# ingonyama-zk/blaze

Measured on AMD Instinct MI355X. Metric: BLS12-381 MSM/s at 2^26, higher is better.
Workload: dtype u32 registers holding 28-bit limbs (381-bit Fq, Montgomery)

## Files before the change

blaze_amd/_lib.py:

```python
from __future__ import annotations

import ctypes as C
import os

_HERE = os.path.dirname(os.path.abspath(__file__))
LIB_PATH = os.environ.get("BLAZE_HIP_LIB") or os.path.join(_HERE, "lib", "libblaze_hip.so")


class DriverClientError(Exception):

    VARIANTS = {
        1: "WriteError",
        2: "ReadError",
        3: "HBICAPNotReady",
        4: "InvalidPrimitiveParam",
        5: "CsvError",
        6: "LoadFailed",
        7: "FileError",
        8: "Unknown",
    }

    def __init__(self, code: int, message: str):
        self.code = code
        self.variant = self.VARIANTS.get(code, "Unknown")
# ... 131 lines not shown
    "blz_poseidon_raw_results": (C.c_int, [C.c_void_p, C.c_uint32, _u8p, C.c_size_t]),
    "blz_poseidon_result": (C.c_int, [C.c_void_p, C.c_uint32, _u8p, C.c_size_t, C.POINTER(C.c_uint32)]),
    "blz_poseidon_tree_device": (C.c_int, [C.c_void_p, C.c_void_p, C.c_size_t]),
    "blz_poseidon_counters": (C.c_int, [C.c_void_p, C.POINTER(C.c_uint32)]),
    "blz_poseidon_info": (C.c_int, [C.c_void_p, C.POINTER(C.c_uint64)]),
    "blz_poseidon_set_round_plan": (C.c_int, [C.c_void_p, C.c_int]),
    "blz_poseidon_prepare_round_plan": (C.c_int, [C.c_void_p, C.POINTER(C.c_uint32)]),
    "blz_poseidon_last_kernel_ms": (C.c_int, [C.c_void_p, C.POINTER(C.c_float)]),
    "blz_poseidon_stream": (C.c_int, [C.c_void_p, C.POINTER(C.c_void_p), C.POINTER(C.c_int)]),
    "blz_poseidon_reset": (C.c_int, [C.c_void_p]),
    "blz_device_malloc": (C.c_int, [C.c_int, C.c_size_t, C.POINTER(C.c_void_p)]),
    "blz_device_free": (C.c_int, [C.c_int, C.c_void_p]),
    "blz_host_malloc": (C.c_int, [C.c_int, C.c_size_t, C.POINTER(C.c_void_p)]),
    "blz_host_free": (C.c_int, [C.c_void_p]),
    "blz_memcpy_h2d": (C.c_int, [C.c_int, C.c_void_p, _u8p, C.c_size_t]),
    "blz_memcpy_d2h": (C.c_int, [C.c_int, _u8p, C.c_void_p, C.c_size_t]),
}
EXPORTED_SYMBOLS = tuple(_SIGS)
_AUX_SIGS = {
    "blz_synth_scalars": (C.c_int, [C.c_int, C.c_int, C.c_void_p, C.c_uint64, C.c_uint64]),
    "blz_synth_scalars_at": (C.c_int, [C.c_int, C.c_int, C.c_void_p, C.c_uint64, C.c_uint64, C.c_uint64]),
    "blz_synth_points": (C.c_int, [C.c_int, C.c_int, C.c_void_p, C.c_uint64, C.c_int, C.c_uint64]),
    "blz_synth_field_elements": (C.c_int, [C.c_int, C.c_void_p, C.c_uint64, C.c_uint64]),
    "blz_calib_mad_rate": (C.c_int, [C.c_int, C.c_uint32, C.POINTER(C.c_double)]),
    "blz_test_msm_stall": (C.c_int, [C.c_void_p, C.c_uint32, C.POINTER(C.c_void_p)]),
    "blz_test_ntt_stall": (C.c_int, [C.c_void_p, C.c_uint32, C.POINTER(C.c_void_p)]),
    "blz_test_stall_release": (C.c_int, [C.c_void_p]),
    "blz_test_field_op": (C.c_int, [C.c_int, C.c_int, C.c_int, C.c_int, _u8p, _u8p, _u8p, C.c_size_t]),
    "blz_test_ec_op": (C.c_int, [C.c_int, C.c_int, C.c_int, _u8p, _u8p, _u8p, _u8p, _u8p, C.c_size_t]),
    "blz_test_msm_tail_plan": (C.c_int, [C.c_int, C.c_int, C.c_uint32, C.c_int, C.c_int, C.c_int, C.c_int, C.c_int, C.POINTER(C.c_uint32), C.POINTER(C.c_uint8),
                                         C.c_char_p, C.c_size_t]),
    "blz_test_msm_sort_plan": (C.c_int, [C.c_int, C.c_int, C.c_uint32, C.c_int, C.c_int, C.c_int, C.c_int, C.c_int, C.c_int, C.c_int, C.c_int, C.c_int,
                                         C.c_char_p, C.c_size_t]),
    "blz_test_law_layout": (C.c_int, [C.c_int, C.c_int, C.c_int, C.POINTER(C.c_uint32)]),
    "blz_test_law_op": (C.c_int, [C.c_int, C.c_int, C.c_int, C.c_int, C.c_int, C.c_int, C.c_uint32, C.c_uint32, _u8p, _u8p, C.c_size_t]),
    "blz_test_rr_layout": (C.c_int, [C.c_int, C.c_int, C.POINTER(C.c_uint32)]),
    "blz_test_rr_op": (C.c_int, [C.c_int, C.c_int, C.c_int, C.c_int, C.c_int, _u8p, _u8p, C.c_size_t]),
    "blz_test_sort_fits_beside": (C.c_int, [C.c_int, C.c_int, C.c_int, C.c_int]),
    "blz_test_poseidon_permute": (C.c_int, [C.c_int, C.c_int, _u8p, C.c_size_t, C.c_int, _u8p, _u8p, C.c_size_t]),
    "blz_test_poseidon_hash": (C.c_int, [C.c_int, C.c_int, _u8p, C.c_size_t, C.c_int, _u8p, _u8p, C.c_size_t]),
    "blz_test_poseidon_hash_plan": (C.c_int, [C.c_int, C.c_int, _u8p, C.c_size_t, C.c_int, _u8p, _u8p, C.c_size_t, C.POINTER(C.c_uint32)]),
    "blz_test_poseidon_tree_check": (C.c_int, [C.c_int, C.c_int, _u8p, C.c_size_t, C.c_int, C.c_uint32, C.c_void_p, C.c_void_p, C.POINTER(C.c_uint64)]),
}
AUX_EXPORTED_SYMBOLS = tuple(_AUX_SIGS)


def lib():
    global _lib
    if _lib is None:
        if not os.path.exists(LIB_PATH):
            raise RuntimeError(
                f"{LIB_PATH} is missing: build it with `make -C blaze_amd/csrc` "
                "(or __graft_entry__.build()); blaze_amd has no CPU fallback"
            )
        L = C.CDLL(LIB_PATH, mode=C.RTLD_GLOBAL)
        for name, (res, args) in _SIGS.items():
            fn = getattr(L, name)
            fn.restype = res
            fn.argtypes = args
        _lib = L
    return _lib


def aux():
    global _aux
    if _aux is None:
# ... 98 lines not shown
```

blaze_amd/csrc/msm_digits.hip.hpp:

```cpp
#pragma once
#include <hip/hip_runtime.h>
#include <cstdint>

namespace blz {

template <int SW>
struct ScalarWords {
    uint32_t s[SW];
    __device__ __forceinline__ void load(const uint32_t* scalars, uint32_t p) {
        if constexpr (SW == 8) {
            const uint4* q = reinterpret_cast<const uint4*>(scalars) + 2 * (size_t)p;
            uint4 a = q[0], b = q[1];
            s[0] = a.x; s[1] = a.y; s[2] = a.z; s[3] = a.w; s[4] = b.x; s[5] = b.y; s[6] = b.z; s[7] = b.w;
        } else if constexpr (SW == 2) {
            const uint2 a = reinterpret_cast<const uint2*>(scalars)[p];
            s[0] = a.x; s[1] = a.y;
        } else {
            s[0] = scalars[p];
        }
    }
    __device__ __forceinline__ int next(int c, uint32_t mask, uint32_t half, uint32_t& carry) {
        uint32_t v = (s[0] & mask) + carry;
#pragma unroll
        for (int i = 0; i + 1 < SW; ++i) s[i] = __builtin_amdgcn_alignbit(s[i + 1], s[i], c);
        s[SW - 1] >>= c;
        if (v > half) { carry = 1; return (int)v - (int)(half << 1); }
        carry = 0;
        return (int)v;
    }
};


#define BLZ_SW_DISPATCH(sbits, ...)                                   \
    do {                                                              \
        if ((sbits) == 256) { constexpr int SW = 8; __VA_ARGS__; }    \
        else if ((sbits) == 64) { constexpr int SW = 2; __VA_ARGS__; } \
        else { constexpr int SW = 1; __VA_ARGS__; }                   \
    } while (0)

}
```

blaze_amd/csrc/msm_engine.hpp:

```cpp
#pragma once
#include "common.hpp"
#include <optional>

namespace blz {

constexpr int MSM_MAX_W = 96;
constexpr uint64_t MSM_MAX_ENTRIES = (1ull << 32) - (1ull << 26);
struct MsmPlan {
    uint32_t npts = 0;
    int sbits = 256;
    int c = 0;
    int W = 0;
    uint8_t width[MSM_MAX_W] = {};
    uint32_t boff[MSM_MAX_W + 1] = {};
    uint32_t Bw = 0;
    int Wv = 0;
    uint64_t G = 0;
    uint32_t L = 0;
    bool table = false;
    int ebits = 0;
    int base_bit = 0;
    double cost = 0;
};
MsmPlan make_plan(uint32_t npts, int sbits, int ebits, int force_c);
// ... 125 lines not shown
    bool can_accept() const;
    MsmPlan plan_for(uint32_t npts, int sbits) const;
    int points_to_mont(const void* d_raw, void* d_mont, uint32_t npts);
    int points_to_mont_even(const void* d_raw, void* d_mont, uint32_t nq);
    int check_precompute(const void* d_raw, uint64_t nelem, uint32_t* flag, hipStream_t st);
    int build_table(const void* d_raw, void* d_table, uint32_t npts, int c, int W, int base_shift, void* scratch, uint32_t* flag,
                    hipStream_t st);
    size_t table_scratch_bytes(int W) const;
    int run(const void* d_points_mont, const void* d_scalars, uint32_t npts, int sbits, int* slot, int table_c = 0, int bit_lo = 0,
            int bit_hi = 0);
    MsmPlan plan_for_range(uint32_t npts, int bit_lo, int bit_hi) const;
    int finish(int slot, uint8_t* out);
    int combine_partials(const uint8_t* partials, size_t count, uint8_t* out, bool on_device);
    int sync_all();
};

struct MsmStep {
    int slot;
    MsmSlot& S;
    int piece;
    const MsmPlan& P;
    MsmEngine::SortBufs& B;
    hipStream_t stream, sort_stream;
};

int msm_points_from_mont(int format_id, const void* d_mont, void* d_raw, uint64_t npts, hipStream_t st);
int msm_points_all_canonical(int format_id, const void* d_raw, uint64_t npts, uint32_t* flag, hipStream_t st);
int copy_words_to_pinned(void* host_pinned, const void* d_src, uint32_t dwords, hipStream_t st);
size_t fq_bytes(int curve);
size_t mont_point_bytes(int curve);
int msm_sort_stage(MsmEngine& E, const MsmStep& C, const void* d_scalars, uint32_t np);
void launch_zero(void* p, size_t n16, hipStream_t st);
bool msm_sort3_ok(const MsmPlan& P, int sbits);
int msm_sort3_max_vgprs(bool table);
int msm_sort3_max_lds(bool table);
bool msm_sort_fits_beside(int av, int sv, int al, int sl);
bool msm_sort_tiny_ok(const MsmPlan& P, uint32_t npts, int sbits);

struct MsmCurveOps {
    int (*points_to_mont)(MsmEngine&, const void* d_raw, void* d_mont, uint32_t npts);
    int (*emit_infinity)(MsmEngine&, int slot);
    int (*run_accumulate)(MsmEngine&, const MsmStep& C, const void* d_pts, uint32_t max_units);
    int (*merge_buckets)(MsmEngine&, const MsmStep& C);
    int (*run_reduce)(MsmEngine&, const MsmStep& C, const void* sums, const void* unit_off);
    TailTraits tail;
    int (*accumulate_vgprs)();
    int (*accumulate_lds)();
    int (*build_table)(MsmEngine&, const void* d_raw, void* d_table, uint32_t npts, int c, int W, int base_shift, void* scratch,
                       uint32_t* flag, hipStream_t st);
    size_t (*table_scratch_bytes)(int W);
    int (*combine)(MsmEngine&, const uint8_t* partials, size_t count, uint8_t* out, bool on_device);
    int (*points_to_mont_even)(MsmEngine&, const void* d_raw, void* d_mont, uint32_t nq);
    int (*check_precompute)(MsmEngine&, const void* d_raw, uint64_t nelem, uint32_t* flag, hipStream_t st);
    int (*points_from_mont)(const void* d_mont, void* d_raw, uint64_t npts, hipStream_t st);
    int (*points_all_canonical)(const void* d_raw, uint64_t npts, uint32_t* flag, hipStream_t st);
};
const MsmCurveOps& msm_ops_bls377();
const MsmCurveOps& msm_ops_bls381();
const MsmCurveOps& msm_ops_bn254();
const MsmCurveOps& msm_ops_bn254_w32();
const MsmCurveOps* msm_ops_for(int curve, int repr = 0);

}
```

blaze_amd/csrc/msm_sort3.hip:

```cpp
#include "msm_sort.hpp"
#include "msm_digits.hip.hpp"

namespace blz {

constexpr int S3_THREADS = 256;
constexpr int S3_SH1 = 14;
constexpr int S3_SH2 = 7;
#ifndef BLZ_S3_T
#define BLZ_S3_T 8
#endif
constexpr int S3_T = BLZ_S3_T;
constexpr int S3_PB = S3_THREADS * S3_T;
constexpr uint32_t S3_SLICE2 = 4096;
constexpr int S3_T2 = S3_SLICE2 / S3_THREADS;
constexpr int S3_T3 = 28;
constexpr uint32_t S3_R3 = S3_THREADS * S3_T3;
constexpr uint32_t S3_MAXNB1 = 2048;
constexpr uint32_t S3_CNT_PTS = 16384;
constexpr uint32_t S3T_IMG = 12288;

struct S3Geom {
    int W, prio;
    uint32_t NB1;
    uint8_t width[MSM_MAX_W];
    uint16_t bitoff[MSM_MAX_W];
    uint16_t binoff1[MSM_MAX_W + 1];
    static constexpr bool TABLE = false;
    static constexpr uint32_t HIST1 = S3_MAXNB1;
    using Win = int;
    __device__ int cw(int w) const { return width[w]; }
    __device__ uint32_t first_bin(int w) const { return binoff1[w]; }
    __device__ static constexpr uint32_t shift1() { return S3_SH1; }
    static constexpr uint32_t bits3() { return S3_SH2; }
    __device__ static uint32_t index1(uint32_t p, uint32_t, uint32_t) { return p; }
    __device__ static uint32_t rem1(uint32_t rem) { return rem; }
    struct L2 {
        int prio;
        using Lo = uint8_t;
        static constexpr uint32_t TAB2 = 128;
        static constexpr uint32_t KY_D = 8, KY_R = 16;
        static constexpr uint32_t LO_MASK = 127u;
        __device__ static constexpr uint32_t shift2() { return S3_SH2; }
        __device__ static constexpr uint32_t bits2() { return S3_SH1 - S3_SH2; }
        __device__ static uint32_t low2(uint32_t r, uint32_t) { return r & 127u; }
        __device__ static uint32_t index2(uint32_t iw) { return iw; }
    };
    L2 l2() const { return L2{prio}; }
};

struct S3TGeom {
    int W, prio, c;
    uint32_t sh1, b2, b3, xs, NB1;
    static constexpr bool TABLE = true;
    static constexpr uint32_t HIST1 = 256;
    using Win = uint32_t;
    __device__ int cw(int) const { return c; }
    __device__ static constexpr uint32_t first_bin(int) { return 0; }
    __device__ uint32_t shift1() const { return sh1; }
    uint32_t bits3() const { return b3; }
    __device__ uint32_t index1(uint32_t p, uint32_t w, uint32_t rem) const { return (p * (uint32_t)W + w) | (xs ? (rem & 1u) << 30 : 0u); }
    __device__ uint32_t rem1(uint32_t rem) const { return rem >> xs; }
    using L2 = S3TGeom;
    using Lo = uint16_t;
    static constexpr uint32_t TAB2 = 256;
    static constexpr uint32_t KY_D = 10, KY_R = 18;
    static constexpr uint32_t LO_MASK = 0x3ffu;
    __device__ uint32_t shift2() const { return b3 - xs; }
    __device__ uint32_t bits2() const { return b2; }
    __device__ uint32_t low2(uint32_t r, uint32_t iw) const {
        const uint32_t lomask = (1u << shift2()) - 1u;
        return xs ? ((r & lomask) << 1) | ((iw >> 30) & 1u) : (r & lomask);
    }
    __device__ static uint32_t index2(uint32_t iw) { return iw & 0xbfffffffu; }
    const L2& l2() const { return *this; }
};

__device__ __forceinline__ void s3_setprio(int p) {
    if (p >= 3) __builtin_amdgcn_s_setprio(3);
    else if (p == 2) __builtin_amdgcn_s_setprio(2);
    else if (p == 1) __builtin_amdgcn_s_setprio(1);
}

__device__ __forceinline__ uint32_t s3_wave_incl_scan(uint32_t v) {
    for (int o = 1; o < 64; o <<= 1) {
        uint32_t t = __shfl_up(v, o, 64);
        if ((threadIdx.x & 63u) >= (uint32_t)o) v += t;
    }
    return v;
}
__device__ __forceinline__ uint32_t s3_block_excl_scan(uint32_t v, uint32_t* wave_tot, uint32_t* total) {
    const uint32_t incl = s3_wave_incl_scan(v);
    if ((threadIdx.x & 63u) == 63u) wave_tot[threadIdx.x >> 6] = incl;
    __syncthreads();
    uint32_t wbase = 0;
    for (uint32_t q = 0; q < (threadIdx.x >> 6); ++q) wbase += wave_tot[q];
    *total = wave_tot[0] + wave_tot[1] + wave_tot[2] + wave_tot[3];
    return wbase + incl - v;
}

template <class Geom, int NW>
__global__ __launch_bounds__(S3_THREADS, 4) void k3_l1_count(const uint32_t* __restrict__ scalars, uint32_t npts, Geom g,
                                                            uint32_t* __restrict__ cnt1) {
    s3_setprio(g.prio);
    __shared__ uint32_t hist[Geom::HIST1];
    if constexpr (Geom::HIST1 == S3_THREADS) hist[threadIdx.x] = 0;
    else for (uint32_t i = threadIdx.x; i < g.NB1; i += S3_THREADS) hist[i] = 0;
    __syncthreads();
    const uint32_t base = blockIdx.x * S3_CNT_PTS;
    uint32_t end = base + S3_CNT_PTS;
    if (end > npts) end = npts;
    for (uint32_t p0 = base + threadIdx.x; p0 < end; p0 += 4 * S3_THREADS) {
        ScalarWords<NW> sw[4];
#pragma unroll
        for (int u = 0; u < 4; ++u) {
            const uint32_t p = p0 + u * S3_THREADS;
            sw[u].load(scalars, p < end ? p : p0);
        }
#pragma unroll
        for (int u = 0; u < 4; ++u) {
            if (p0 + u * S3_THREADS >= end) break;
            uint32_t carry = 0;
            for (int w = 0; w < g.W; ++w) {
                const int cw = g.cw(w);
                const int d = sw[u].next(cw, (1u << cw) - 1u, 1u << (cw - 1), carry);
                if (d != 0) {
                    const uint32_t b = (uint32_t)(d < 0 ? -d : d) - 1u;
                    atomicAdd(&hist[g.first_bin(w) + (b >> g.shift1())], 1u);
                }
            }
        }
    }
    __syncthreads();
    auto flush = [&](uint32_t i) {
        const uint32_t v = hist[i];
        if (v) atomicAdd(&cnt1[i], v);
    };
    if constexpr (Geom::HIST1 == S3_THREADS) { if (threadIdx.x < g.NB1) flush(threadIdx.x); }
    else for (uint32_t i = threadIdx.x; i < g.NB1; i += S3_THREADS) flush(i);
}

__global__ __launch_bounds__(S3_THREADS) void k3_scan_small(const uint32_t* __restrict__ cnt, uint32_t n, uint32_t* __restrict__ off,
                                                           uint32_t* __restrict__ cur, int prio) {
    s3_setprio(prio);
    __shared__ uint32_t wave_tot[4];
    uint32_t v[8], sum = 0;
    const uint32_t b0 = threadIdx.x * 8u;
#pragma unroll
    for (int k = 0; k < 8; ++k) {
        v[k] = b0 + k < n ? cnt[b0 + k] : 0u;
        sum += v[k];
    }
    uint32_t total;
    uint32_t run = s3_block_excl_scan(sum, wave_tot, &total);
#pragma unroll
    for (int k = 0; k < 8; ++k) {
        if (b0 + k < n) {
            off[b0 + k] = run;
            cur[b0 + k] = run;
        }
        run += v[k];
    }
    if (threadIdx.x == 0) off[n] = total;
}

template <class Geom, int NW>
__global__ __launch_bounds__(S3_THREADS, 4) void k3_l1_scatter(const uint32_t* __restrict__ scalars, uint32_t npts, Geom g,
                                                              uint32_t* __restrict__ cur1, uint32_t* __restrict__ o_idx,
                                                              uint16_t* __restrict__ o_rem) {
    s3_setprio(g.prio);
    extern __shared__ __attribute__((aligned(16))) uint32_t sh[];
    uint32_t* sc = sh;
    uint2* stage = reinterpret_cast<uint2*>(sh + NW * S3_PB);
    uint32_t* hist = sh + (NW + 2) * S3_PB;
    uint32_t* lstart = hist + 256;
    uint32_t* gbase = lstart + 256;
    __shared__ uint32_t wave_tot[4];
    const uint32_t tid = threadIdx.x;
    const uint32_t base = blockIdx.x * (uint32_t)S3_PB;
#pragma unroll
    for (int u = 0; u < S3_T; ++u) {
        const uint32_t p = base + u * S3_THREADS + tid;
        const uint32_t i = u * S3_THREADS + tid;
        if constexpr (NW == 8) {
            uint4 a = make_uint4(0, 0, 0, 0), b = make_uint4(0, 0, 0, 0);
            if (p < npts) {
                const uint4* q = reinterpret_cast<const uint4*>(scalars) + 2 * (size_t)p;
                a = q[0];
                b = q[1];
            }
            sc[0 * S3_PB + i] = a.x; sc[1 * S3_PB + i] = a.y; sc[2 * S3_PB + i] = a.z; sc[3 * S3_PB + i] = a.w;
            sc[4 * S3_PB + i] = b.x; sc[5 * S3_PB + i] = b.y; sc[6 * S3_PB + i] = b.z; sc[7 * S3_PB + i] = b.w;
        } else if constexpr (NW == 2) {
            uint2 a = make_uint2(0, 0);
            if (p < npts) a = reinterpret_cast<const uint2*>(scalars)[p];
            sc[0 * S3_PB + i] = a.x; sc[1 * S3_PB + i] = a.y;
        } else {
            sc[i] = p < npts ? scalars[p] : 0u;
        }
    }
    uint32_t carry = 0;
    using Win = typename Geom::Win;
    for (Win w = 0; w < (Win)g.W; ++w) {
        uint32_t cw, off, nb;
        if constexpr (Geom::TABLE) { cw = (uint32_t)g.c; off = w * cw; nb = g.NB1; }
        else { cw = g.width[w]; off = g.bitoff[w]; nb = (uint32_t)g.binoff1[w + 1] - (uint32_t)g.binoff1[w]; }
        const uint32_t sh1 = g.shift1(), lowmask = (1u << sh1) - 1u;
        const uint32_t j = off >> 5, shb = off & 31u, mask = (1u << cw) - 1u, half = 1u << (cw - 1);
        if (Geom::TABLE || tid < nb) hist[tid] = 0;
        __syncthreads();
        uint32_t key[S3_T], rk[S3_T];
#pragma unroll
        for (int u = 0; u < S3_T; ++u) {
            const uint32_t i = u * S3_THREADS + tid;
            const uint32_t lo = j < (uint32_t)NW ? sc[j * S3_PB + i] : 0u;
            const uint32_t hi = j + 1 < (uint32_t)NW ? sc[(j + 1) * S3_PB + i] : 0u;
            const uint32_t raw = (shb ? __builtin_amdgcn_alignbit(hi, lo, shb) : lo) & mask;
            const uint32_t v = raw + ((carry >> u) & 1u);
            int d;
            if (v > half) { d = (int)v - (int)(half << 1); carry |= 1u << u; }
            else { d = (int)v; carry &= ~(1u << u); }
            rk[u] = ~0u;
            key[u] = 0;
            if (d != 0 && base + i < npts) {
                const uint32_t b = (uint32_t)(d < 0 ? -d : d) - 1u;
                const uint32_t bin = b >> sh1;
                key[u] = (b & lowmask) | (bin << sh1) | (d < 0 ? 0x80000000u : 0u);
                rk[u] = atomicAdd(&hist[bin], 1u);
            }
        }
        __syncthreads();
        {
            const uint32_t v = tid < nb ? hist[tid] : 0u;
            uint32_t total;
            const uint32_t excl = s3_block_excl_scan(v, wave_tot, &total);
            if (tid < nb) {
                lstart[tid] = excl;
                uint32_t ci;
                if constexpr (Geom::TABLE) ci = tid; else ci = (uint32_t)g.binoff1[w] + tid;
                gbase[tid] = v ? atomicAdd(&cur1[ci], v) : 0u;
            }
            __syncthreads();
#pragma unroll
            for (int u = 0; u < S3_T; ++u) {
                if (rk[u] != ~0u) {
                    const uint32_t bin = (key[u] >> sh1) & (Geom::TABLE ? 0xffu : 0x1ffu);
                    const uint32_t p = base + u * S3_THREADS + tid;
                    const uint32_t rem = key[u] & lowmask;
                    stage[lstart[bin] + rk[u]] = make_uint2((Geom::TABLE ? g.index1(p, (uint32_t)w, rem) : p) | (key[u] & 0x80000000u), g.rem1(rem) | (bin << 16));
                }
            }
            __syncthreads();
            for (uint32_t slot = tid; slot < total; slot += S3_THREADS) {
                const uint2 e = stage[slot];
                const uint32_t bin = e.y >> 16;
                const uint32_t dst = gbase[bin] + (slot - lstart[bin]);
                o_idx[dst] = e.x;
                o_rem[dst] = (uint16_t)e.y;
            }
        }
        __syncthreads();
    }
}

__global__ __launch_bounds__(S3_THREADS) void k3_slice_map(const uint32_t* __restrict__ off, uint32_t nbins, uint32_t slice,
                                                          uint2* __restrict__ map, uint32_t* __restrict__ nitems, int prio) {
    s3_setprio(prio);
    __shared__ uint32_t wave_tot[4];
    __shared__ uint32_t carry_sh;
    if (threadIdx.x == 0) carry_sh = 0;
    __syncthreads();
    for (uint32_t base = 0; base < nbins; base += S3_THREADS) {
        const uint32_t i = base + threadIdx.x;
        const uint32_t size = i < nbins ? off[i + 1] - off[i] : 0u;
        const uint32_t v = (size + slice - 1) / slice;
        uint32_t total;
        const uint32_t excl = s3_block_excl_scan(v, wave_tot, &total);
        const uint32_t first = carry_sh + excl;
        for (uint32_t q = 0; q < v; ++q) map[first + q] = make_uint2(i, q);
        __syncthreads();
        if (threadIdx.x == 0) carry_sh += total;
        __syncthreads();
    }
    if (threadIdx.x == 0) *nitems = carry_sh;
}

__global__ __launch_bounds__(S3_THREADS) void k3_scan_a(const uint32_t* __restrict__ cnt, uint32_t n, uint32_t* __restrict__ bsum, int prio) {
    s3_setprio(prio);
    __shared__ uint32_t wave_tot[4];
    const uint32_t b0 = blockIdx.x * 2048u + threadIdx.x * 8u;
    uint32_t sum = 0;
#pragma unroll
    for (int k = 0; k < 8; ++k) sum += b0 + k < n ? cnt[b0 + k] : 0u;
    uint32_t total;
// ... 79 lines not shown
    s3_setprio(g.prio);
    constexpr uint32_t TAB2 = Geom::TAB2, KY_D = Geom::KY_D, KY_R = Geom::KY_R;
    __shared__ uint2 stage[S3_SLICE2];
    __shared__ uint32_t hist[TAB2], lstart[TAB2], gbase[TAB2];
    __shared__ uint32_t wave_tot[4];
    uint32_t k, lo, hi;
    if (!s3_item(off1, map, nitems, blockIdx.x, S3_SLICE2, k, lo, hi)) return;
    const uint32_t tid = threadIdx.x;
    if (TAB2 == S3_THREADS || tid < TAB2) hist[tid] = 0;
    __syncthreads();
    const uint32_t sh = g.shift2(), nb2 = 1u << g.bits2();
    uint32_t ex[S3_T2], ky[S3_T2];
#pragma unroll
    for (int t = 0; t < S3_T2; ++t) {
        const uint32_t i = lo + t * S3_THREADS + tid;
        ky[t] = 0xffffffffu;
        ex[t] = 0;
        if (i < hi) {
            const uint32_t r = i_rem[i];
            const uint32_t iw = i_idx[i];
            const uint32_t h2 = r >> sh;
            const uint32_t low = g.low2(r, iw);
            ex[t] = g.index2(iw);
            const uint32_t rank = atomicAdd(&hist[h2], 1u);
            ky[t] = low | (h2 << KY_D) | (rank << KY_R);
        }
    }
    __syncthreads();
    const uint32_t v = tid < nb2 ? hist[tid] : 0u;
    uint32_t total;
    const uint32_t excl = s3_block_excl_scan(v, wave_tot, &total);
    if (tid < nb2) {
        lstart[tid] = excl;
        gbase[tid] = v ? atomicAdd(&cur2[(k << g.bits2()) + tid], v) : 0u;
    }
    __syncthreads();
#pragma unroll
    for (int t = 0; t < S3_T2; ++t) {
        if (ky[t] != 0xffffffffu) {
            const uint32_t h2 = (ky[t] >> KY_D) & (TAB2 - 1u);
            stage[lstart[h2] + (ky[t] >> KY_R)] = make_uint2(ex[t], ky[t] & ((TAB2 << KY_D) - 1u));
        }
    }
    __syncthreads();
    for (uint32_t slot = tid; slot < total; slot += S3_THREADS) {
        const uint2 e = stage[slot];
        const uint32_t h2 = (e.y >> KY_D) & (TAB2 - 1u);
        const uint32_t dst = gbase[h2] + (slot - lstart[h2]);
        o_idx[dst] = e.x;
        o_lo[dst] = (typename Geom::Lo)(e.y & Geom::LO_MASK);
    }
}

__global__ __launch_bounds__(S3_THREADS, 4) void k3_l3(const uint32_t* __restrict__ i_idx, const uint8_t* __restrict__ i_lo,
                                                      const uint32_t* __restrict__ off2, uint32_t* __restrict__ count,
                                                      uint32_t* __restrict__ entries, int prio) {
    s3_setprio(prio);
    __shared__ uint32_t out[S3_R3];
    __shared__ uint32_t hist[128], cursor[128];
    __shared__ uint32_t wave_tot[4];
    const uint32_t j = blockIdx.x, tid = threadIdx.x;
    const uint32_t a = off2[j], b = off2[j + 1], s = b - a;
    if (tid < 128) hist[tid] = 0;
    __syncthreads();
    if (s <= S3_R3) {
        uint32_t ex[S3_T3], ky[S3_T3];
#pragma unroll
        for (int t = 0; t < S3_T3; ++t) {
            const uint32_t i = a + t * S3_THREADS + tid;
            ky[t] = 0xffffffffu;
            ex[t] = 0;
            if (i < b) {
                ky[t] = i_lo[i];
                ex[t] = i_idx[i];
            }
        }
#pragma unroll
        for (int t = 0; t < S3_T3; ++t)
            if (ky[t] != 0xffffffffu) ky[t] |= atomicAdd(&hist[ky[t]], 1u) << 8;
        __syncthreads();
        const uint32_t v = tid < 128 ? hist[tid] : 0u;
// ... 143 lines not shown
    g.W = P.W;
    g.prio = exp_knob("BLAZE_SORT_PRIO", 3);
    g.NB1 = (uint32_t)(P.G >> S3_SH1);
    uint32_t bit = 0;
    for (int w = 0; w < P.W; ++w) {
        g.width[w] = P.width[w];
        g.bitoff[w] = (uint16_t)bit;
        g.binoff1[w] = (uint16_t)(P.boff[w] >> S3_SH1);
        bit += P.width[w];
    }
    g.binoff1[P.W] = (uint16_t)(P.boff[P.W] >> S3_SH1);
    return g;
}

static S3TGeom s3t_geometry(const MsmPlan& P, uint32_t npts) {
    S3TGeom g;
    g.W = P.W;
    g.c = P.c;
    g.prio = exp_knob("BLAZE_SORT_PRIO", 3);
    g.sh1 = (uint32_t)(P.c - 1 - 8);
    g.NB1 = (uint32_t)(P.G >> g.sh1);
    const double per_bucket = (double)npts * P.W / (double)P.G;
    int b3 = 4;
    while (b3 < 10 && (double)(2u << b3) * per_bucket <= 6144.0) ++b3;
    if ((uint32_t)b3 > g.sh1) b3 = (int)g.sh1;
    int b2 = (int)g.sh1 - b3;
    if (b2 > 8) { b2 = 8; b3 = (int)g.sh1 - 8; }
    g.b2 = (uint32_t)b2;
    g.b3 = (uint32_t)b3;
    g.xs = g.sh1 > 16 ? g.sh1 - 16 : 0;
    return g;
}

bool msm_sort3_ok(const MsmPlan& P, int sbits) {
    if (P.table) {
        if (sbits != 256 || P.sbits < 1 || P.sbits > 256 || P.c < 16 || P.c > 26 || P.W * P.c < P.sbits + 1) return false;
        if ((uint64_t)P.npts * P.W >= (1ull << 30)) return false;
        const S3TGeom g = s3t_geometry(P, P.npts);
        return g.NB1 <= 256 && g.b2 <= 8 && g.b3 >= 1 && g.b3 <= 10 && g.xs <= 1 && g.b3 > g.xs;
    }
    if ((sbits != 256 && sbits != 64 && sbits != 32) || P.W < 1) return false;
    for (int w = 0; w < P.W; ++w)
        if (P.width[w] < S3_SH1 + 1 || P.width[w] > 23) return false;
    if ((P.G >> S3_SH1) > S3_MAXNB1 || (P.G & ((1u << S3_SH1) - 1u))) return false;
    if ((P.G >> S3_SH2) > 2048u * 256u) return false;
    return true;
}

static constexpr size_t s3_lds1(int nw) { return (size_t)((nw + 2) * S3_PB + 3 * 256) * 4; }
struct S3Need { int vgprs, lds; };
static S3Need s3_needs(bool table) {
    using L2 = S3Geom::L2;
    struct K { const void* f; size_t dyn; };
    static const K plain_ks[] = {{(const void*)k3_l1_count<S3Geom, 8>, 0}, {(const void*)k3_l1_scatter<S3Geom, 8>, s3_lds1(8)},
                                 {(const void*)k3_l1_count<S3Geom, 1>, 0}, {(const void*)k3_l1_scatter<S3Geom, 1>, s3_lds1(1)},
                                 {(const void*)k3_l1_count<S3Geom, 2>, 0}, {(const void*)k3_l1_scatter<S3Geom, 2>, s3_lds1(2)},
                                 {(const void*)k3_l2_count<L2>, 0}, {(const void*)k3_l2_scatter<L2>, 0}, {(const void*)k3_l3, 0}};
    static const K table_ks[] = {{(const void*)k3_l1_count<S3TGeom, 8>, 0}, {(const void*)k3_l1_scatter<S3TGeom, 8>, s3_lds1(8)},
                                 {(const void*)k3_l2_count<S3TGeom>, 0}, {(const void*)k3_l2_scatter<S3TGeom>, 0},
                                 {(const void*)k3t_l3<true>, (size_t)S3_R3 * 4}, {(const void*)k3t_l3<false>, (size_t)S3T_IMG * 4}};
    static S3Need cached[2] = {{-1, -1}, {-1, -1}};
    S3Need& c = cached[table ? 1 : 0];
    if (c.vgprs >= 0) return c;
    const K* ks = table ? table_ks : plain_ks;
    const size_t n = table ? sizeof(table_ks) / sizeof(*table_ks) : sizeof(plain_ks) / sizeof(*plain_ks);
    S3Need mx = {0, 0};
    for (size_t i = 0; i < n; ++i) {
        hipFuncAttributes a;
        if (hipFuncGetAttributes(&a, ks[i].f) != hipSuccess) {
            (void)hipGetLastError();
            return c = S3Need{0, 0};
        }
        if (a.numRegs > mx.vgprs) mx.vgprs = a.numRegs;
        const int lds = (int)(a.sharedSizeBytes + ks[i].dyn);
// ... 50 lines not shown
    const uint32_t* sc = (const uint32_t*)d_scalars;
    const dim3 blk(S3_THREADS);
    const L2 g2 = g.l2();

    BLZ_HIP(hipMemsetAsync(cnt1, 0, (size_t)(NB1 + 2) * 4, st), BLZ_ERR_UNKNOWN);
    BLZ_HIP(hipMemsetAsync(cnt2, 0, (size_t)(NB2 + 2) * 4, st), BLZ_ERR_UNKNOWN);
    if constexpr (Geom::TABLE) {
        BLZ_TRY((s3_level1<Geom, 8>(st, sc, npts, g, cnt1, off1, cur1, i1_idx, i1_rem)));
    } else {
        BLZ_SW_DISPATCH(sbits, BLZ_TRY((s3_level1<Geom, SW>(st, sc, npts, g, cnt1, off1, cur1, i1_idx, i1_rem))));
    }
    hipLaunchKernelGGL(k3_slice_map, dim3(1), blk, 0, st, off1, NB1, S3_SLICE2, map, nitems, g.prio);
    hipLaunchKernelGGL(k3_l2_count<L2>, dim3(max_items), blk, 0, st, i1_rem, off1, map, nitems, cnt2, g2);
    hipLaunchKernelGGL(k3_scan_a, dim3(nsb), blk, 0, st, cnt2, NB2, bsum, g.prio);
    hipLaunchKernelGGL(k3_scan_b, dim3(1), blk, 0, st, bsum, nsb, g.prio);
    hipLaunchKernelGGL(k3_scan_c, dim3(nsb), blk, 0, st, cnt2, NB2, bsum, off2, cur2, g.prio);
    hipLaunchKernelGGL(k3_l2_scatter<L2>, dim3(max_items), blk, 0, st, i1_idx, i1_rem, off1, map, nitems, cur2, i2_idx, i2_lo, g2);
    if constexpr (Geom::TABLE) {
        const double mean_bin = (double)max_entries / (double)(NB2 ? NB2 : 1);
        const bool big_bins = mean_bin * 1.1 > (double)S3_R3;
        const uint32_t img = big_bins ? S3T_IMG : S3_R3;
        auto l3 = big_bins ? k3t_l3<false> : k3t_l3<true>;
        BLZ_TRY(ensure_dynamic_lds((const void*)l3, (int)(img * 4)));
        hipLaunchKernelGGL(l3, dim3(NB2), blk, (size_t)img * 4, st, i2_idx, i2_lo, off2, count, entries, g, img);
    } else {
        hipLaunchKernelGGL(k3_l3, dim3(NB2), blk, 0, st, i2_idx, i2_lo, off2, count, entries, g.prio);
    }
    BLZ_HIP(hipGetLastError(), BLZ_ERR_UNKNOWN);
    return BLZ_OK;
}

int msm_sort3(MsmEngine& E, const MsmStep& C, const void* d_scalars, uint32_t npts, int sbits) {
    const MsmPlan& P = C.P;
    return P.table ? s3_enqueue(E, C, s3t_geometry(P, P.npts), d_scalars, npts, sbits) : s3_enqueue(E, C, s3_geometry(P), d_scalars, npts, sbits);
}

}
```

blaze_amd/csrc/testhooks.hip:

```cpp
#include "common.hpp"
#include "ec_rr.hip.hpp"
#include "ec_row.hip.hpp"
#include "ec_law.hip.hpp"
#include "poseidon_engine.hpp"
#include "poseidon_impl.hip.hpp"
#include "msm_engine.hpp"
#include "../../include/blaze_hip_aux.h"

namespace blz {

template <class P>
__global__ __launch_bounds__(64) void k_test_field(int op, const uint32_t* a, const uint32_t* b, uint32_t* out, uint32_t n) {
    uint32_t i = blockIdx.x * 64u + threadIdx.x;
    if (i >= n) return;
    Fp<P> x, y, r;
    fp_load(x, a + (size_t)i * P::N);
    fp_load(y, b + (size_t)i * P::N);
    fp_to_mont(x, x);
    fp_to_mont(y, y);
    switch (op) {
        case 0: fp_mul(r, x, y); break;
        case 1: fp_add(r, x, y); break;
        case 2: fp_sub(r, x, y); break;
        case 3: fp_inv(r, x); break;
// ... 1241 lines not shown
                           uint8_t* widths, char* text, size_t cap) {
    if (!plan_out || !text || cap == 0) return fail(BLZ_ERR_INVALID_PARAM, "null argument");
    const MsmCurveOps* ops = msm_ops_for(curve, repr);
    if (!ops || npts == 0) return fail(BLZ_ERR_INVALID_PARAM, "unknown curve %d or empty task", curve);
    MsmPlan P;
    BLZ_TRY(msm_task_plan(curve, npts, sbits, table_c, bit_lo, bit_hi, P, nullptr));
    uint32_t per = 0;
    pieces = msm_task_pieces(P, pieces, false, &per);
    TailPlan T;
    BLZ_TRY(plan_tail(P, ops->tail, pieces > 1, T));
    const uint32_t out[8] = {(uint32_t)P.c, (uint32_t)P.W, (uint32_t)P.G, P.L, P.Bw, (uint32_t)P.Wv, (uint32_t)P.ebits, P.table ? 1u : 0u};
    memcpy(plan_out, out, sizeof(out));
    if (widths) memcpy(widths, P.width, (size_t)P.W);
    const std::string line = describe(T);
    if (line.size() >= cap) return fail(BLZ_ERR_INVALID_PARAM, "text buffer of %zu bytes for a line of %zu", cap, line.size());
    memcpy(text, line.c_str(), line.size() + 1);
    return BLZ_OK;
}

int blz_test_msm_sort_plan(int curve, int repr, uint32_t npts, int sbits, int pieces, int table_c, int bit_lo, int bit_hi, int hide_env, int other_busy,
                           int recent_hot, int fits, char* text, size_t cap) {
    if (!text || cap == 0) return fail(BLZ_ERR_INVALID_PARAM, "null argument");
    if (!msm_ops_for(curve, repr) || npts == 0) return fail(BLZ_ERR_INVALID_PARAM, "unknown curve %d or empty task", curve);
    MsmPlan P;
    BLZ_TRY(msm_task_plan(curve, npts, sbits, table_c, bit_lo, bit_hi, P, nullptr));
    uint32_t per = 0;
    pieces = msm_task_pieces(P, pieces, false, &per);
    const std::string line = describe(plan_sort(P, npts, sbits, pieces, SortInputs{hide_env, other_busy != 0, recent_hot != 0, fits != 0}));
    if (line.size() >= cap) return fail(BLZ_ERR_INVALID_PARAM, "text buffer of %zu bytes for a line of %zu", cap, line.size());
    memcpy(text, line.c_str(), line.size() + 1);
    return BLZ_OK;
}

int blz_test_law_layout(int curve, int repr, int law, uint32_t out[32]) {
    if (!out) return fail(BLZ_ERR_INVALID_PARAM, "null argument");
    LawLayout L;
    BLZ_TRY(test_law_dispatch(curve, repr, law, &L, nullptr));
    memset(out, 0, 32 * sizeof(uint32_t));
    const uint32_t head[6] = {L.B, L.NL, L.stride, L.e, L.lanes, L.closed};
    memcpy(out, head, sizeof(head));
    const LawBound* b[4] = {&L.in, &L.store, &L.strict, &L.to_lane};
    for (int i = 0; i < 4; ++i) memcpy(out + 6 + 5 * i, b[i], sizeof(LawBound));
    out[26] = L.tree ? 1u : 0u;
    return BLZ_OK;
}

int blz_test_law_op(int device_id, int curve, int repr, int law, int program, int exit, uint32_t k, uint32_t arg, const uint32_t* in, uint32_t* out,
                    size_t n) {
    if (!in || !out) return fail(BLZ_ERR_INVALID_PARAM, "null argument");
    LawLayout L;
    BLZ_TRY(test_law_dispatch(curve, repr, law, &L, nullptr));
    if (program < 0 || program >= LAW_PROGRAMS) return fail(BLZ_ERR_INVALID_PARAM, "unknown program %d", program);
    if (program == LAW_TREE) {
        if (!L.tree) return fail(BLZ_ERR_INVALID_PARAM, "the shuffle tree runs on the reduced-radix lane law only");
        if (k < 1 || k > 64 || arg < 1 || arg > k) return fail(BLZ_ERR_INVALID_PARAM, "tree of %u lanes over %u points", arg, k);
    } else {
        if (k != 4) return fail(BLZ_ERR_INVALID_PARAM, "program %d takes 4 points per case, not %u", program, k);
        if (arg > 64) return fail(BLZ_ERR_INVALID_PARAM, "%u doublings per step (at most 64)", arg);
    }
    const LawBound& ex = exit == 0 ? L.store : exit == 1 ? L.to_lane : L.strict;
    if (exit < 0 || exit > 2 || ex.limb_max == 0) return fail(BLZ_ERR_INVALID_PARAM, "law %d has no exit %d", law, exit);
    if (n == 0) return BLZ_OK;
    if (n > (1u << 20)) return fail(BLZ_ERR_INVALID_PARAM, "%zu cases (at most 2^20)", n);
    BLZ_TRY(use_device(device_id));
    const LawOp op = {program, exit, k, arg, in, out, n};
    return test_law_dispatch(curve, repr, law, nullptr, &op);
// ... 21 lines not shown
```

include/blaze_hip_aux.h:

```cpp
#ifndef BLAZE_HIP_AUX_H
#define BLAZE_HIP_AUX_H

#include "blaze_hip.h"

#ifdef __cplusplus
extern "C" {
#endif


int blz_synth_scalars(int device_id, int curve, void* d_out, uint64_t n, uint64_t seed);
int blz_synth_scalars_at(int device_id, int curve, void* d_out, uint64_t n, uint64_t seed, uint64_t start);
int blz_synth_points(int device_id, int curve, void* d_out, uint64_t n, int pf, uint64_t start);
int blz_synth_field_elements(int device_id, void* d_out, uint64_t n, uint64_t seed);

int blz_calib_mad_rate(int device_id, uint32_t target_ms, double out[4]);

int blz_test_msm_stall(blz_msm* h, uint32_t max_ms, void** token);
int blz_test_ntt_stall(blz_ntt* h, uint32_t max_ms, void** token);
int blz_test_stall_release(void* token);

int blz_test_field_op(int device_id, int curve, int field, int op, const uint8_t* a, const uint8_t* b,
                      uint8_t* out, size_t n);
int blz_test_ec_op(int device_id, int curve, int op, const uint8_t* p, const uint8_t* q,
                   const uint8_t* inf_flags, uint8_t* out, uint8_t* out_inf, size_t n);

int blz_test_msm_tail_plan(int curve, int repr, uint32_t npts, int sbits, int pieces, int table_c, int bit_lo, int bit_hi, uint32_t plan_out[8],
                           uint8_t* widths, char* text, size_t cap);
int blz_test_msm_sort_plan(int curve, int repr, uint32_t npts, int sbits, int pieces, int table_c, int bit_lo, int bit_hi, int hide_env, int other_busy,
                           int recent_hot, int fits, char* text, size_t cap);

int blz_test_law_layout(int curve, int repr, int law, uint32_t out[32]);
int blz_test_law_op(int device_id, int curve, int repr, int law, int program, int exit, uint32_t k, uint32_t arg, const uint32_t* in,
                    uint32_t* out, size_t n);

#define BLZ_RR_LAYOUT_WORDS 8192
int blz_test_rr_layout(int curve, int field, uint32_t* out);
int blz_test_rr_op(int device_id, int curve, int field, int op, int variant, const uint32_t* in, uint32_t* out, size_t n);

int blz_test_sort_fits_beside(int acc_vgprs, int sort_vgprs, int acc_lds, int sort_lds);

int blz_test_poseidon_permute(int device_id, int field, const uint8_t* words, size_t len, int t, const uint8_t* states_in,
                              uint8_t* states_out, size_t n);
int blz_test_poseidon_hash(int device_id, int field, const uint8_t* words, size_t len, int t, const uint8_t* inputs, uint8_t* digests,
                           size_t n);
int blz_test_poseidon_hash_plan(int device_id, int field, const uint8_t* words, size_t len, int t, const uint8_t* inputs, uint8_t* digests,
                                size_t n, uint32_t* state);
int blz_test_poseidon_tree_check(int device_id, int field, const uint8_t* words, size_t len, int tree_mode, uint32_t tree_height,
                                 const void* d_input, const void* d_records, uint64_t out[2]);

#ifdef __cplusplus
}
#endif
#endif
```

Baseline: 8.297.

## Replace sequential signed-digit carry chain with precomputed digit bias in sort3

Signed-window digits are obtained by adding a precomputed bias constant (the sum of 2^(c-1)-1 for each window) to the scalar once. Each digit then becomes an independent extract-and-subtract, which removes the serial carry propagation across windows in the count and scatter kernels. The scatter kernel also skips windows beyond the scalar data when no wave carries out, zeroes the histogram inside the scan, folds the local-start offset into gbase, and drops one block barrier per window. This adds a plan-validity check that can reject plans whose windows extend past the bias words, and relies on the barrier removal being safe.

```diff
diff --git a/blaze_amd/_lib.py b/blaze_amd/_lib.py
--- a/blaze_amd/_lib.py
+++ b/blaze_amd/_lib.py
@@ -187,6 +187,7 @@
                                          C.c_char_p, C.c_size_t]),
     "blz_test_msm_sort_plan": (C.c_int, [C.c_int, C.c_int, C.c_uint32, C.c_int, C.c_int, C.c_int, C.c_int, C.c_int, C.c_int, C.c_int, C.c_int, C.c_int,
                                          C.c_char_p, C.c_size_t]),
+    "blz_test_msm_digit_bias": (C.c_int, [C.c_int, C.c_int, C.c_uint32, C.c_int, C.c_int, C.POINTER(C.c_uint32), C.POINTER(C.c_uint8)]),
     "blz_test_law_layout": (C.c_int, [C.c_int, C.c_int, C.c_int, C.POINTER(C.c_uint32)]),
     "blz_test_law_op": (C.c_int, [C.c_int, C.c_int, C.c_int, C.c_int, C.c_int, C.c_int, C.c_uint32, C.c_uint32, _u8p, _u8p, C.c_size_t]),
     "blz_test_rr_layout": (C.c_int, [C.c_int, C.c_int, C.POINTER(C.c_uint32)]),
diff --git a/blaze_amd/csrc/msm_digits.hip.hpp b/blaze_amd/csrc/msm_digits.hip.hpp
--- a/blaze_amd/csrc/msm_digits.hip.hpp
+++ b/blaze_amd/csrc/msm_digits.hip.hpp
@@ -4,9 +4,27 @@
 
 namespace blz {
 
+struct DigitBias {
+    uint32_t lo[8];
+    uint32_t hi[2];
+    int nd;
+};
+__device__ __forceinline__ int biased_digit(uint32_t lo, uint32_t hi, uint32_t shb, uint32_t mask, uint32_t hm1) {
+    return (int)(__builtin_amdgcn_alignbit(hi, lo, shb) & mask) - (int)hm1;
+}
+__device__ __forceinline__ uint32_t biased_word_above(const DigitBias& b, uint32_t k, uint32_t c) {
+    return k == 0 ? b.hi[0] + c : k == 1 ? b.hi[1] : 0u;
+}
+
 template <int SW>
 struct ScalarWords {
     uint32_t s[SW];
+    __device__ __forceinline__ uint32_t add_bias(const DigitBias& b) {
+        uint32_t c = 0;
+#pragma unroll
+        for (int i = 0; i < SW; ++i) s[i] = __builtin_addc(s[i], b.lo[i], c, &c);
+        return c;
+    }
     __device__ __forceinline__ void load(const uint32_t* scalars, uint32_t p) {
         if constexpr (SW == 8) {
             const uint4* q = reinterpret_cast<const uint4*>(scalars) + 2 * (size_t)p;
diff --git a/blaze_amd/csrc/msm_engine.hpp b/blaze_amd/csrc/msm_engine.hpp
--- a/blaze_amd/csrc/msm_engine.hpp
+++ b/blaze_amd/csrc/msm_engine.hpp
@@ -181,6 +181,7 @@
 int msm_sort_stage(MsmEngine& E, const MsmStep& C, const void* d_scalars, uint32_t np);
 void launch_zero(void* p, size_t n16, hipStream_t st);
 bool msm_sort3_ok(const MsmPlan& P, int sbits);
+bool msm_sort3_digit_bias(const MsmPlan& P, int sbits, uint32_t words[10], int* data_windows);
 int msm_sort3_max_vgprs(bool table);
 int msm_sort3_max_lds(bool table);
 bool msm_sort_fits_beside(int av, int sv, int al, int sl);
diff --git a/blaze_amd/csrc/msm_sort3.hip b/blaze_amd/csrc/msm_sort3.hip
--- a/blaze_amd/csrc/msm_sort3.hip
+++ b/blaze_amd/csrc/msm_sort3.hip
@@ -25,6 +25,7 @@
     uint8_t width[MSM_MAX_W];
     uint16_t bitoff[MSM_MAX_W];
     uint16_t binoff1[MSM_MAX_W + 1];
+    DigitBias bias;
     static constexpr bool TABLE = false;
     static constexpr uint32_t HIST1 = S3_MAXNB1;
     using Win = int;
@@ -51,6 +52,7 @@
 struct S3TGeom {
     int W, prio, c;
     uint32_t sh1, b2, b3, xs, NB1;
+    DigitBias bias;
     static constexpr bool TABLE = true;
     static constexpr uint32_t HIST1 = 256;
     using Win = uint32_t;
@@ -109,23 +111,50 @@
     const uint32_t base = blockIdx.x * S3_CNT_PTS;
     uint32_t end = base + S3_CNT_PTS;
     if (end > npts) end = npts;
+    const uint32_t sh1 = g.shift1();
     for (uint32_t p0 = base + threadIdx.x; p0 < end; p0 += 4 * S3_THREADS) {
         ScalarWords<NW> sw[4];
+        uint32_t top[4];
 #pragma unroll
         for (int u = 0; u < 4; ++u) {
             const uint32_t p = p0 + u * S3_THREADS;
-            sw[u].load(scalars, p < end ? p : p0);
+#pragma unroll
+            for (int i = 0; i < NW; ++i) sw[u].s[i] = 0;
+            if (p < end) sw[u].load(scalars, p);
+            top[u] = g.bias.hi[0] + sw[u].add_bias(g.bias);
+        }
+        int w = 0;
+#pragma unroll
+        for (int j = 0; j < NW; ++j) {
+            for (; w < g.bias.nd; ++w) {
+                uint32_t cw, off;
+                if constexpr (Geom::TABLE) { cw = (uint32_t)g.c; off = (uint32_t)w * cw; }
+                else { cw = g.width[w]; off = g.bitoff[w]; }
+                if (off >= 32u * (j + 1)) break;
+                const uint32_t shb = off & 31u, mask = (1u << cw) - 1u, hm1 = (1u << (cw - 1)) - 1u, fb = g.first_bin(w);
+#pragma unroll
+                for (int u = 0; u < 4; ++u) {
+                    const int d = biased_digit(sw[u].s[j], j + 1 < NW ? sw[u].s[(j + 1) % NW] : top[u], shb, mask, hm1);
+                    if (d != 0) {
+                        const uint32_t b = (uint32_t)(d < 0 ? -d : d) - 1u;
+                        atomicAdd(&hist[fb + (b >> sh1)], 1u);
+                    }
+                }
+            }
         }
 #pragma unroll
         for (int u = 0; u < 4; ++u) {
-            if (p0 + u * S3_THREADS >= end) break;
-            uint32_t carry = 0;
-            for (int w = 0; w < g.W; ++w) {
-                const int cw = g.cw(w);
-                const int d = sw[u].next(cw, (1u << cw) - 1u, 1u << (cw - 1), carry);
+            if (top[u] == g.bias.hi[0]) continue;
+            for (int wc = g.bias.nd; wc < g.W; ++wc) {
+                const uint32_t cw = (uint32_t)g.cw(wc);
+                uint32_t off;
+                if constexpr (Geom::TABLE) off = (uint32_t)wc * cw; else off = g.bitoff[wc];
+                const uint32_t k = (off >> 5) - (uint32_t)NW;
+                const int d = biased_digit(biased_word_above(g.bias, k, 1u), biased_word_above(g.bias, k + 1, 1u), off & 31u, (1u << cw) - 1u,
+                                           (1u << (cw - 1)) - 1u);
                 if (d != 0) {
                     const uint32_t b = (uint32_t)(d < 0 ? -d : d) - 1u;
-                    atomicAdd(&hist[g.first_bin(w) + (b >> g.shift1())], 1u);
+                    atomicAdd(&hist[g.first_bin(wc) + (b >> sh1)], 1u);
                 }
             }
         }
@@ -169,75 +198,75 @@
                                                               uint16_t* __restrict__ o_rem) {
     s3_setprio(g.prio);
     extern __shared__ __attribute__((aligned(16))) uint32_t sh[];
-    uint32_t* sc = sh;
-    uint2* stage = reinterpret_cast<uint2*>(sh + NW * S3_PB);
-    uint32_t* hist = sh + (NW + 2) * S3_PB;
+    uint32_t* hist = sh;
     uint32_t* lstart = hist + 256;
     uint32_t* gbase = lstart + 256;
+    uint32_t* sc = sh + 3 * 256;
+    uint2* stage = reinterpret_cast<uint2*>(sc + NW * S3_PB);
     __shared__ uint32_t wave_tot[4];
     const uint32_t tid = threadIdx.x;
     const uint32_t base = blockIdx.x * (uint32_t)S3_PB;
+    __shared__ uint32_t wave_carry[4];
+    uint32_t carry = 0;
 #pragma unroll
     for (int u = 0; u < S3_T; ++u) {
         const uint32_t p = base + u * S3_THREADS + tid;
         const uint32_t i = u * S3_THREADS + tid;
-        if constexpr (NW == 8) {
-            uint4 a = make_uint4(0, 0, 0, 0), b = make_uint4(0, 0, 0, 0);
-            if (p < npts) {
-                const uint4* q = reinterpret_cast<const uint4*>(scalars) + 2 * (size_t)p;
-                a = q[0];
-                b = q[1];
-            }
-            sc[0 * S3_PB + i] = a.x; sc[1 * S3_PB + i] = a.y; sc[2 * S3_PB + i] = a.z; sc[3 * S3_PB + i] = a.w;
-            sc[4 * S3_PB + i] = b.x; sc[5 * S3_PB + i] = b.y; sc[6 * S3_PB + i] = b.z; sc[7 * S3_PB + i] = b.w;
-        } else if constexpr (NW == 2) {
-            uint2 a = make_uint2(0, 0);
-            if (p < npts) a = reinterpret_cast<const uint2*>(scalars)[p];
-            sc[0 * S3_PB + i] = a.x; sc[1 * S3_PB + i] = a.y;
-        } else {
-            sc[i] = p < npts ? scalars[p] : 0u;
-        }
-    }
-    uint32_t carry = 0;
+        ScalarWords<NW> sw;
+#pragma unroll
+        for (int k = 0; k < NW; ++k) sw.s[k] = 0;
+        if (p < npts) sw.load(scalars, p);
+        carry |= sw.add_bias(g.bias) << u;
+#pragma unroll
+        for (int k = 0; k < NW; ++k) sc[k * S3_PB + i] = sw.s[k];
+    }
+    const uint32_t wave_carries = __any(carry != 0) ? 1u : 0u;
+    if ((tid & 63u) == 0) wave_carry[tid >> 6] = wave_carries;
+    hist[tid] = 0;
+    __syncthreads();
     using Win = typename Geom::Win;
     for (Win w = 0; w < (Win)g.W; ++w) {
+        if (w >= (Win)g.bias.nd && !__builtin_amdgcn_readfirstlane(wave_carry[0] | wave_carry[1] | wave_carry[2] | wave_carry[3])) break;
         uint32_t cw, off, nb;
         if constexpr (Geom::TABLE) { cw = (uint32_t)g.c; off = w * cw; nb = g.NB1; }
         else { cw = g.width[w]; off = g.bitoff[w]; nb = (uint32_t)g.binoff1[w + 1] - (uint32_t)g.binoff1[w]; }
         const uint32_t sh1 = g.shift1(), lowmask = (1u << sh1) - 1u;
-        const uint32_t j = off >> 5, shb = off & 31u, mask = (1u << cw) - 1u, half = 1u << (cw - 1);
-        if (Geom::TABLE || tid < nb) hist[tid] = 0;
-        __syncthreads();
+        const uint32_t j = off >> 5, shb = off & 31u, mask = (1u << cw) - 1u, hm1 = (1u << (cw - 1)) - 1u;
         uint32_t key[S3_T], rk[S3_T];
-#pragma unroll
-        for (int u = 0; u < S3_T; ++u) {
-            const uint32_t i = u * S3_THREADS + tid;
-            const uint32_t lo = j < (uint32_t)NW ? sc[j * S3_PB + i] : 0u;
-            const uint32_t hi = j + 1 < (uint32_t)NW ? sc[(j + 1) * S3_PB + i] : 0u;
-            const uint32_t raw = (shb ? __builtin_amdgcn_alignbit(hi, lo, shb) : lo) & mask;
-            const uint32_t v = raw + ((carry >> u) & 1u);
-            int d;
-            if (v > half) { d = (int)v - (int)(half << 1); carry |= 1u << u; }
-            else { d = (int)v; carry &= ~(1u << u); }
+        auto rank = [&](int u, uint32_t lo, uint32_t hi) {
+            const int d = biased_digit(lo, hi, shb, mask, hm1);
+            const uint32_t b = (uint32_t)(d < 0 ? -d : d) - 1u;
+            key[u] = b | ((uint32_t)d & 0x80000000u);
             rk[u] = ~0u;
-            key[u] = 0;
-            if (d != 0 && base + i < npts) {
-                const uint32_t b = (uint32_t)(d < 0 ? -d : d) - 1u;
-                const uint32_t bin = b >> sh1;
-                key[u] = (b & lowmask) | (bin << sh1) | (d < 0 ? 0x80000000u : 0u);
-                rk[u] = atomicAdd(&hist[bin], 1u);
+            if (d != 0) rk[u] = atomicAdd(&hist[b >> sh1], 1u);
+        };
+        if (j + 1 < (uint32_t)NW) {
+#pragma unroll
+            for (int u = 0; u < S3_T; ++u) {
+                const uint32_t i = u * S3_THREADS + tid;
+                rank(u, sc[j * S3_PB + i], sc[(j + 1) * S3_PB + i]);
+            }
+        } else {
+            const uint32_t ulo = j < (uint32_t)NW ? 0u : biased_word_above(g.bias, j - NW, 0u), clo = j == (uint32_t)NW ? 1u : 0u;
+            const uint32_t uhi = biased_word_above(g.bias, j + 1 - NW, 0u), chi = j + 1 == (uint32_t)NW ? 1u : 0u;
+#pragma unroll
+            for (int u = 0; u < S3_T; ++u) {
+                const uint32_t i = u * S3_THREADS + tid;
+                const uint32_t cb = (carry >> u) & 1u;
+                rank(u, j < (uint32_t)NW ? sc[j * S3_PB + i] : ulo + (cb & clo), uhi + (cb & chi));
             }
         }
         __syncthreads();
         {
-            const uint32_t v = tid < nb ? hist[tid] : 0u;
+            const uint32_t v = hist[tid];
+            hist[tid] = 0;
             uint32_t total;
             const uint32_t excl = s3_block_excl_scan(v, wave_tot, &total);
             if (tid < nb) {
                 lstart[tid] = excl;
                 uint32_t ci;
                 if constexpr (Geom::TABLE) ci = tid; else ci = (uint32_t)g.binoff1[w] + tid;
-                gbase[tid] = v ? atomicAdd(&cur1[ci], v) : 0u;
+                gbase[tid] = (v ? atomicAdd(&cur1[ci], v) : 0u) - excl;
             }
             __syncthreads();
 #pragma unroll
@@ -252,13 +281,11 @@
             __syncthreads();
             for (uint32_t slot = tid; slot < total; slot += S3_THREADS) {
                 const uint2 e = stage[slot];
-                const uint32_t bin = e.y >> 16;
-                const uint32_t dst = gbase[bin] + (slot - lstart[bin]);
+                const uint32_t dst = gbase[e.y >> 16] + slot;
                 o_idx[dst] = e.x;
                 o_rem[dst] = (uint16_t)e.y;
             }
         }
-        __syncthreads();
     }
 }
 
@@ -404,7 +431,7 @@
     const uint32_t excl = s3_block_excl_scan(v, wave_tot, &total);
     if (tid < nb2) {
         lstart[tid] = excl;
-        gbase[tid] = v ? atomicAdd(&cur2[(k << g.bits2()) + tid], v) : 0u;
+        gbase[tid] = (v ? atomicAdd(&cur2[(k << g.bits2()) + tid], v) : 0u) - excl;
     }
     __syncthreads();
 #pragma unroll
@@ -418,7 +445,7 @@
     for (uint32_t slot = tid; slot < total; slot += S3_THREADS) {
         const uint2 e = stage[slot];
         const uint32_t h2 = (e.y >> KY_D) & (TAB2 - 1u);
-        const uint32_t dst = gbase[h2] + (slot - lstart[h2]);
+        const uint32_t dst = gbase[h2] + slot;
         o_idx[dst] = e.x;
         o_lo[dst] = (typename Geom::Lo)(e.y & Geom::LO_MASK);
     }
@@ -628,14 +655,41 @@
     return g;
 }
 
+static bool s3_bias(const MsmPlan& P, int sbits, DigitBias& B) {
+    const int nw = sbits / 32;
+    uint32_t h[10] = {};
+    B.nd = 0;
+    uint32_t off = 0;
+    for (int w = 0; w < P.W; ++w) {
+        const uint32_t cw = P.width[w];
+        if (off + cw > 32u * nw + 64u) return false;
+        for (uint32_t bit = off; bit + 1 < off + cw; ++bit) h[bit >> 5] |= 1u << (bit & 31u);
+        if (off < 32u * nw) B.nd = w + 1;
+        off += cw;
+    }
+    for (int i = 0; i < 8; ++i) B.lo[i] = i < nw ? h[i] : 0u;
+    B.hi[0] = h[nw];
+    B.hi[1] = h[nw + 1];
+    return true;
+}
+bool msm_sort3_digit_bias(const MsmPlan& P, int sbits, uint32_t words[10], int* data_windows) {
+    DigitBias B;
+    if (!msm_sort3_ok(P, sbits) || !s3_bias(P, sbits, B)) return false;
+    memcpy(words, B.lo, sizeof(B.lo));
+    memcpy(words + 8, B.hi, sizeof(B.hi));
+    *data_windows = B.nd;
+    return true;
+}
+
 bool msm_sort3_ok(const MsmPlan& P, int sbits) {
+    DigitBias B;
+    if ((sbits != 256 && sbits != 64 && sbits != 32) || P.W < 1 || P.W > MSM_MAX_W || !s3_bias(P, sbits, B)) return false;
     if (P.table) {
         if (sbits != 256 || P.sbits < 1 || P.sbits > 256 || P.c < 16 || P.c > 26 || P.W * P.c < P.sbits + 1) return false;
         if ((uint64_t)P.npts * P.W >= (1ull << 30)) return false;
         const S3TGeom g = s3t_geometry(P, P.npts);
         return g.NB1 <= 256 && g.b2 <= 8 && g.b3 >= 1 && g.b3 <= 10 && g.xs <= 1 && g.b3 > g.xs;
     }
-    if ((sbits != 256 && sbits != 64 && sbits != 32) || P.W < 1) return false;
     for (int w = 0; w < P.W; ++w)
         if (P.width[w] < S3_SH1 + 1 || P.width[w] > 23) return false;
     if ((P.G >> S3_SH1) > S3_MAXNB1 || (P.G & ((1u << S3_SH1) - 1u))) return false;
@@ -752,7 +806,14 @@
 
 int msm_sort3(MsmEngine& E, const MsmStep& C, const void* d_scalars, uint32_t npts, int sbits) {
     const MsmPlan& P = C.P;
-    return P.table ? s3_enqueue(E, C, s3t_geometry(P, P.npts), d_scalars, npts, sbits) : s3_enqueue(E, C, s3_geometry(P), d_scalars, npts, sbits);
-}
-
-}
+    if (P.table) {
+        S3TGeom g = s3t_geometry(P, P.npts);
+        if (!s3_bias(P, sbits, g.bias)) return fail(BLZ_ERR_UNKNOWN, "three-level sort: the plan's windows reach beyond the digit bias");
+        return s3_enqueue(E, C, g, d_scalars, npts, sbits);
+    }
+    S3Geom g = s3_geometry(P);
+    if (!s3_bias(P, sbits, g.bias)) return fail(BLZ_ERR_UNKNOWN, "three-level sort: the plan's windows reach beyond the digit bias");
+    return s3_enqueue(E, C, g, d_scalars, npts, sbits);
+}
+
+}
diff --git a/blaze_amd/csrc/testhooks.hip b/blaze_amd/csrc/testhooks.hip
--- a/blaze_amd/csrc/testhooks.hip
+++ b/blaze_amd/csrc/testhooks.hip
@@ -1297,6 +1297,21 @@
     return BLZ_OK;
 }
 
+int blz_test_msm_digit_bias(int curve, int repr, uint32_t npts, int sbits, int table_c, uint32_t out[14], uint8_t* widths) {
+    if (!out || !widths) return fail(BLZ_ERR_INVALID_PARAM, "null argument");
+    if (!msm_ops_for(curve, repr) || npts == 0) return fail(BLZ_ERR_INVALID_PARAM, "unknown curve %d or empty task", curve);
+    MsmPlan P;
+    BLZ_TRY(msm_task_plan(curve, npts, sbits, table_c, 0, 0, P, nullptr));
+    int nd = 0;
+    if (!msm_sort3_digit_bias(P, sbits, out + 4, &nd)) return fail(BLZ_ERR_INVALID_PARAM, "the three-level sort does not take this plan");
+    out[0] = (uint32_t)P.W;
+    out[1] = (uint32_t)(sbits / 32);
+    out[2] = (uint32_t)nd;
+    out[3] = P.table ? 1u : 0u;
+    memcpy(widths, P.width, (size_t)P.W);
+    return BLZ_OK;
+}
+
 int blz_test_law_layout(int curve, int repr, int law, uint32_t out[32]) {
     if (!out) return fail(BLZ_ERR_INVALID_PARAM, "null argument");
     LawLayout L;
diff --git a/include/blaze_hip_aux.h b/include/blaze_hip_aux.h
--- a/include/blaze_hip_aux.h
+++ b/include/blaze_hip_aux.h
@@ -28,6 +28,7 @@
                            uint8_t* widths, char* text, size_t cap);
 int blz_test_msm_sort_plan(int curve, int repr, uint32_t npts, int sbits, int pieces, int table_c, int bit_lo, int bit_hi, int hide_env, int other_busy,
                            int recent_hot, int fits, char* text, size_t cap);
+int blz_test_msm_digit_bias(int curve, int repr, uint32_t npts, int sbits, int table_c, uint32_t out[14], uint8_t* widths);
 
 int blz_test_law_layout(int curve, int repr, int law, uint32_t out[32]);
 int blz_test_law_op(int device_id, int curve, int repr, int law, int program, int exit, uint32_t k, uint32_t arg, const uint32_t* in,
```

Result: no change. 8.325 (median of 6 runs) (+0.3%).
